# Glaciohound/Chimera-ST

Measured on AMD Instinct MI355X. Metric: train utterances/sec, MuST-C EN-DE s2t_transformer_m, 1/2/4/8 MI355X, higher is better.
Workload: dtype bf16

## Files before the change

chimera-st_amd/csrc/gemm.hip:

```cpp
#include "gemm_common.h"
#include <vector>
#include <stdlib.h>
#include <string>
#include <type_traits>

namespace {
using namespace cstg;

template <int BM_, int BN_, int WM_, int WN_, int KV_ = 8>
struct Cfg {
  static constexpr int BM = BM_, BN = BN_, WM = WM_, WN = WN_, NT = 64 * WM_ * WN_, TM = BM_ / WM_ / 32, TN = BN_ / WN_ / 32;
  static constexpr int KV = KV_;
  static_assert(BM_ <= GEMM_MAX_BM && GEMM_MAX_BM % BM_ == 0, "conv0.hip (cst_conv_row_limits) sizes live frames from GEMM_MAX_BM");
};
using CfgSmall = Cfg<128, 128, 2, 2>;
using CfgSkinny = Cfg<64, 64, 2, 2>;
using CfgNarrowN = Cfg<128, 64, 2, 2>;
using CfgNarrowM = Cfg<64, 128, 2, 2>;
using CfgLarge = Cfg<256, 256, 4, 4>;

template <typename T, bool A_KMAJOR, bool B_KMAJOR, bool SEG, typename C, bool CS = false>
__global__ __launch_bounds__(C::NT) void gemm_kernel(GemmParams p) {
  constexpr int BM = C::BM, BN = C::BN, NTHREADS = C::NT, TM = C::TM, TN = C::TN;
  constexpr int VEC = DT<T>::VEC;
// ... 698 lines not shown
      for (; sp < p.splits; ++sp) {
        const f32x4 a0 = *reinterpret_cast<const f32x4*>(src + (int64_t)sp * total), a1 = *reinterpret_cast<const f32x4*>(src + (int64_t)sp * total + 4);
#pragma unroll
        for (int e = 0; e < 4; ++e) { v[e] += a0[e]; v[4 + e] += a1[e]; }
      }
      const int64_t i = i8 * 8, row = i / p.N;
      epilogue_store8<T>(p, cofs, bofs, row, i - row * p.N, v);
    }
    return;
  }
  for (int64_t i = (int64_t)blockIdx.x * blockDim.x + threadIdx.x; i < total; i += (int64_t)gridDim.x * blockDim.x) {
    float v = 0.0f;
    for (int s = 0; s < p.splits; ++s) v += ws[s * total + i];
    epilogue_store<T>(p, cofs, bofs, i / p.N, i % p.N, v);
  }
}

template <typename T, bool AK, bool BK_, bool SEG, typename C>
int launch(GemmParams p, int64_t M, int64_t N, int64_t nbatch, hipStream_t s) {
  constexpr int VEC = DT<T>::VEC;
  constexpr int BKc = C::KV * VEC, LDK = BKc + VEC;
  constexpr int LDMA = sizeof(T) == 2 ? C::BM + 32 : C::BM + VEC, LDMB = sizeof(T) == 2 ? C::BN + 32 : C::BN + VEC;
  constexpr int A_ELEMS = AK ? C::BM * LDK : BKc * LDMA;
  constexpr int B_ELEMS = BK_ ? C::BN * LDK : BKc * LDMB;
  size_t lds = 2 * (size_t)(A_ELEMS + B_ELEMS) * sizeof(T);
  const size_t stage_bytes = (size_t)64 * (C::BN + 4) * sizeof(float);
  if (lds < stage_bytes) lds = stage_bytes;
  static bool attr_set = false;
  if (!attr_set) {
    (void)hipFuncSetAttribute(reinterpret_cast<const void*>(&gemm_kernel<T, AK, BK_, SEG, C>), hipFuncAttributeMaxDynamicSharedMemorySize, 160 * 1024 - 4096);
    attr_set = true;
  }
  p.tiles_m = (int)cst_ceil_div(M, C::BM);
  p.tiles_n = (int)cst_ceil_div(N, C::BN);
  static const bool no_split_order = getenv("CST_GEMM_NO_SPLIT_ORDER") != nullptr;
  p.split_order = (p.splits > 1 && nbatch == 1 && !no_split_order) ? 1 : 0;
  dim3 grid(p.tiles_m * p.tiles_n, 1, (unsigned)(nbatch * p.splits));
  if constexpr (!AK && !BK_ && !SEG && C::NT <= 256) {
    if (p.colsum) {
      static bool attr_cs = false;
      if (!attr_cs) {
        (void)hipFuncSetAttribute(reinterpret_cast<const void*>(&gemm_kernel<T, AK, BK_, SEG, C, true>), hipFuncAttributeMaxDynamicSharedMemorySize, 160 * 1024 - 4096);
        attr_cs = true;
      }
      hipLaunchKernelGGL((gemm_kernel<T, AK, BK_, SEG, C, true>), grid, dim3(C::NT), lds, s, p);
      return cst_check_launch("cst_gemm");
    }
  }
  if (p.colsum) { cst_set_error("cst_gemm: internal: column sums requested from a configuration that does not build them"); return CST_ERR_UNSUPPORTED; }
  hipLaunchKernelGGL((gemm_kernel<T, AK, BK_, SEG, C>), grid, dim3(C::NT), lds, s, p);
  return cst_check_launch("cst_gemm");
}

template <typename T, bool AK, bool BK_, typename C, int NS>
int launch_glds(GemmParams p, int64_t M, int64_t N, int64_t nbatch, hipStream_t s) {
  constexpr int ES = sizeof(T), BKc = 128 / ES;
  constexpr int A_BYTES = AK ? C::BM * 128 : BKc * C::BM * ES, B_BYTES = BK_ ? C::BN * 128 : BKc * C::BN * ES;
  size_t lds = (size_t)NS * (A_BYTES + B_BYTES);
  const size_t stage_bytes = (size_t)64 * (C::BN + 4) * sizeof(float);
  if (lds < stage_bytes) lds = stage_bytes;
  static bool attr_set = false;
  if (!attr_set) {
    (void)hipFuncSetAttribute(reinterpret_cast<const void*>(&gemm_glds_kernel<T, AK, BK_, C, NS>), hipFuncAttributeMaxDynamicSharedMemorySize, 160 * 1024);
    attr_set = true;
  }
  p.tiles_m = (int)cst_ceil_div(M, C::BM);
  p.tiles_n = (int)cst_ceil_div(N, C::BN);
  dim3 grid(p.tiles_m * p.tiles_n, 1, (unsigned)(nbatch * p.splits));
  hipLaunchKernelGGL((gemm_glds_kernel<T, AK, BK_, C, NS>), grid, dim3(C::NT), lds, s, p);
  return cst_check_launch("cst_gemm");
}

bool use_large(const cst_gemm_desc* d, int splits) {
  if ((d->a_kmajor && d->a_seg) || (d->b_kmajor && d->b_seg)) return false;
  const int64_t tiles = cst_ceil_div(d->M, 256) * cst_ceil_div(d->N, 256) * d->batch0 * d->batch1 * splits;
  return d->M >= 256 && d->N >= 256 && tiles >= 200;
}

bool getenv_no_glds() {
  static const bool v = getenv("CST_GEMM_NO_GLDS") != nullptr;
  return v;
}

int choose_splits(const cst_gemm_desc* d) {
  if (d->split_k > 1) return d->split_k;
  if (d->split_k == 0 || d->split_k == 1) return 1;
  const int bk = d->dtype == CST_BF16 ? 64 : 32;
  const int64_t ktiles = cst_ceil_div(d->K, bk);
  const int64_t nb = d->batch0 * d->batch1;
  if (d->M >= 256 && d->N >= 256) {
    const int64_t tl = cst_ceil_div(d->M, 256) * cst_ceil_div(d->N, 256) * nb;
    if (tl >= 200) return 1;
    int64_t s = 256 / tl;
    if (s > ktiles / 16) s = ktiles / 16;
    if (s > 32) s = 32;
    if (s >= 1 && tl * s >= 200) return (int)s;
  }
  const int64_t tiles = cst_ceil_div(d->M, 128) * cst_ceil_div(d->N, 128) * nb;
  if (tiles >= 256 || ktiles < 16) return 1;
  const int64_t cap = ktiles / 8 < 32 ? ktiles / 8 : 32;
  int64_t s1 = 256 / tiles, s2 = 512 / tiles;
  if (s1 > cap) s1 = cap;
  if (s2 > cap) s2 = cap;
  if (s1 < 1) s1 = 1;
  if (s2 < 1) s2 = 1;
  const int64_t s = (2.0 / (double)s2 < 0.9 / (double)s1) ? s2 : s1;
  return (int)s;
}

}

static bool colsum_fused(const cst_gemm_desc* d, int splits) {
  return d->colsum && !d->a_kmajor && !d->b_kmajor && !d->a_seg && !d->b_seg && !use_large(d, splits);
}

extern "C" int64_t cst_colsum_workspace(int64_t rows, int64_t cols);
extern "C" int cst_colsum_typed(const void* x, int64_t ldx, void* out, void* workspace, int64_t rows, int64_t cols, int dtype, int out_dtype, cst_stream stream);
extern "C" int cst_colsum_typed_live(const void* x, int64_t ldx, void* out, void* workspace, int64_t rows, int64_t cols, int dtype, int out_dtype,
                                     const uint32_t* row_live, uint32_t epoch, cst_stream stream);

extern "C" int cst_gemm_splits(const cst_gemm_desc* d) { return d ? choose_splits(d) : 0; }

extern "C" int cst_gemm_colsum_is_fused(const cst_gemm_desc* d) { return d && colsum_fused(d, choose_splits(d)) ? 1 : 0; }

extern "C" int64_t cst_gemm_workspace(const cst_gemm_desc* d) {
  const int s = choose_splits(d);
  const int64_t nb = d->batch0 * d->batch1;
  int64_t bytes = s > 1 ? (int64_t)s * d->M * d->N * nb * (int64_t)sizeof(float) : 0;
  if (d->colsum) bytes += colsum_fused(d, s) ? (s > 1 ? (int64_t)s * d->M * nb * (int64_t)sizeof(float) : 0) : cst_colsum_workspace(d->K, d->M);
  return bytes;
}

static int gemm_one(const cst_gemm_desc* d, cst_stream stream, int64_t drop_row0) {
  CST_REQUIRE(d && d->A && d->B && d->C, "cst_gemm: null operand");
  CST_REQUIRE(d->dtype == CST_F32 || d->dtype == CST_BF16, "cst_gemm: bad dtype %d", d->dtype);
  CST_REQUIRE(d->c_dtype == d->dtype || d->c_dtype == CST_F32, "cst_gemm: c_dtype must be dtype or f32");
  CST_REQUIRE(d->M > 0 && d->N > 0 && d->K > 0, "cst_gemm: empty problem M=%lld N=%lld K=%lld", (long long)d->M,
              (long long)d->N, (long long)d->K);
  const int vec = d->dtype == CST_BF16 ? 8 : 4;
  if (d->a_kmajor) CST_REQUIRE(d->K % vec == 0 && d->lda % vec == 0, "cst_gemm: k-major A needs K,lda %% %d == 0 (K=%lld lda=%lld)", vec, (long long)d->K, (long long)d->lda);
  else CST_REQUIRE(d->M % vec == 0 && d->lda % vec == 0, "cst_gemm: mn-major A needs M,lda %% %d == 0 (M=%lld lda=%lld)", vec, (long long)d->M, (long long)d->lda);
  if (d->b_kmajor) CST_REQUIRE(d->K % vec == 0 && d->ldb % vec == 0, "cst_gemm: k-major B needs K,ldb %% %d == 0 (K=%lld ldb=%lld)", vec, (long long)d->K, (long long)d->ldb);
  else CST_REQUIRE(d->N % vec == 0 && d->ldb % vec == 0, "cst_gemm: mn-major B needs N,ldb %% %d == 0 (N=%lld ldb=%lld)", vec, (long long)d->N, (long long)d->ldb);
  CST_REQUIRE(d->a_seg % vec == 0 && d->b_seg % vec == 0 && d->a_seg_stride % vec == 0 && d->b_seg_stride % vec == 0,
              "cst_gemm: segment sizes must be multiples of %d", vec);
  CST_REQUIRE(((uintptr_t)d->A % 16 == 0) && ((uintptr_t)d->B % 16 == 0), "cst_gemm: A/B must be 16-byte aligned");
  CST_REQUIRE(d->sa0 % vec == 0 && d->sa1 % vec == 0 && d->sb0 % vec == 0 && d->sb1 % vec == 0, "cst_gemm: batch strides of A/B must be multiples of %d", vec);
  CST_REQUIRE(d->batch0 >= 1 && d->batch1 >= 1, "cst_gemm: batch counts must be >= 1");
  CST_REQUIRE(!d->dact || d->aux_in, "cst_gemm: dact needs aux_in");

  GemmParams p;
  p.M = d->M; p.N = d->N; p.K = d->K;
  p.A = d->A; p.lda = d->lda; p.a_seg = d->a_seg; p.a_seg_stride = d->a_seg_stride;
  p.B = d->B; p.ldb = d->ldb; p.b_seg = d->b_seg; p.b_seg_stride = d->b_seg_stride;
  p.C = d->C; p.ldc = d->ldc;
  p.bias = d->bias; p.bias_mode = d->bias ? d->bias_mode : CST_BIAS_NONE; p.sbias0 = d->sbias0; p.sbias1 = d->sbias1;
  p.act = d->act;
  p.aux_out = d->aux_out; p.ld_aux_out = d->ld_aux_out;
  p.dact = d->dact; p.aux_in = d->aux_in; p.ld_aux_in = d->ld_aux_in;
  p.resid = d->resid; p.ld_resid = d->ld_resid;
  p.alpha = d->alpha;
  CST_REQUIRE(d->drop_p >= 0.0f && d->drop_p < 1.0f, "cst_gemm: drop_p must be in [0, 1)");
  CST_REQUIRE(d->drop_p == 0.0f || d->batch0 * d->batch1 == 1, "cst_gemm: fused dropout needs an unbatched problem");
  p.drop_thr = d->drop_p > 0.0f ? cst_drop_thr16(d->drop_p) : 0u;
  p.drop_key = d->drop_key;
  p.drop_scale = d->drop_p > 0.0f ? 1.0f / (1.0f - d->drop_p) : 1.0f;
  p.drop_row0 = drop_row0;
  p.batch1 = d->batch1;
  p.sa0 = d->sa0; p.sa1 = d->sa1; p.sb0 = d->sb0; p.sb1 = d->sb1; p.sc0 = d->sc0; p.sc1 = d->sc1;
  p.c_f32 = (d->c_dtype == CST_F32 && d->dtype != CST_F32) ? 1 : 0;
  if (d->dtype == CST_F32) p.c_f32 = 0;
  {
    auto al16 = [](const void* q) { return q == nullptr || ((uintptr_t)q % 16) == 0; };
    bool ok = d->ldc % 8 == 0 && d->sc0 % 8 == 0 && d->sc1 % 8 == 0 && al16(d->C) && al16(d->bias) && al16(d->aux_out) && al16(d->aux_in) && al16(d->resid);
    if (d->bias && d->bias_mode == CST_BIAS_COL) ok = ok && d->sbias0 % 8 == 0 && d->sbias1 % 8 == 0;
    if (d->aux_out) ok = ok && d->ld_aux_out % 8 == 0;
    if (d->aux_in) ok = ok && d->ld_aux_in % 8 == 0;
    if (d->resid) ok = ok && d->ld_resid % 8 == 0;
    if (d->drop_p > 0.0f) ok = ok && (d->N % 2 == 0);
    p.vec_epi = ok ? 1 : 0;
  }
  p.tiles_m = p.tiles_n = 0;
  p.split_order = 0;
  p.sched = nullptr;
  p.gperm_full = 0;
  p.mrot = 0;
  {
    static const bool no_klive = getenv("CST_GEMM_NO_KLIVE") != nullptr;
    p.k_live = no_klive ? nullptr : d->k_live;
    p.k_epoch = d->k_epoch;
    p.m_live = no_klive ? nullptr : d->m_live;
    p.m_epoch = d->m_epoch;
    p.k_len = no_klive ? nullptr : d->k_len;
    p.m_len = no_klive ? nullptr : d->m_len;
  }
  {
    static const int gm = getenv("CST_GEMM8P_GROUP_M") ? atoi(getenv("CST_GEMM8P_GROUP_M")) : 4;
    p.group_m = gm > 0 ? gm : 4;
  }
  p.splits = choose_splits(d);
  p.ws = nullptr;
  CST_REQUIRE(!d->colsum || (!d->a_kmajor && !d->a_seg), "cst_gemm: colsum needs an mn-major, unsegmented A");
  const bool cs_fused = colsum_fused(d, p.splits);
  CST_REQUIRE(!d->colsum || cs_fused || (d->batch0 * d->batch1 == 1 && d->M % 8 == 0 && d->lda % 8 == 0),
              "cst_gemm: colsum of this configuration runs as a separate column sum: unbatched, M and lda multiples of 8");
  p.colsum = cs_fused ? d->colsum : nullptr;
  p.colsum_ws = nullptr;
#ifdef CST_TRACE
  if (p.splits == 1 && d->workspace) p.ws = (float*)d->workspace;
#endif
  const int64_t nbatch = d->batch0 * d->batch1;
  CST_REQUIRE(cst_ceil_div(d->M, 128) * cst_ceil_div(d->N, 128) < (1ll << 31) && nbatch * p.splits < 65536, "cst_gemm: grid too large");
  if (p.splits > 1) {
    const int64_t need = cst_gemm_workspace(d);
    if (!d->workspace || d->workspace_bytes < need) {
      cst_set_error("cst_gemm: split_k=%d needs %lld workspace bytes, got %lld", p.splits, (long long)need,
                    (long long)d->workspace_bytes);
      return CST_ERR_WORKSPACE;
    }
    p.ws = (float*)d->workspace;
    p.colsum_ws = p.ws + (int64_t)p.splits * d->M * d->N * nbatch;
  } else if (d->colsum && !cs_fused && (!d->workspace || d->workspace_bytes < cst_gemm_workspace(d))) {
    cst_set_error("cst_gemm: colsum needs %lld workspace bytes, got %lld", (long long)cst_gemm_workspace(d), (long long)d->workspace_bytes);
    return CST_ERR_WORKSPACE;
  }
  hipStream_t s = (hipStream_t)stream;
  double kfrac = 1.0;
  if (p.k_live && cst_prof_is_on()) {
    const int64_t nt = cst_ceil_div(d->K, 64);
    std::vector<uint32_t> st((size_t)nt);
    if (hipStreamSynchronize(s) == hipSuccess && hipMemcpy(st.data(), p.k_live, sizeof(uint32_t) * nt, hipMemcpyDeviceToHost) == hipSuccess) {
      int64_t live = 0;
      for (int64_t i = 0; i < nt; ++i) live += st[i] == p.k_epoch;
      kfrac = (double)live / (double)nt;
    }
  }
  if (p.k_len && cst_prof_is_on()) {
    std::vector<int32_t> kl((size_t)d->batch0);
    if (hipStreamSynchronize(s) == hipSuccess && hipMemcpy(kl.data(), p.k_len, sizeof(int32_t) * d->batch0, hipMemcpyDeviceToHost) == hipSuccess) {
      double sum = 0.0;
      for (int64_t b = 0; b < d->batch0; ++b) sum += (double)(kl[b] < 0 ? 0 : (kl[b] < d->K ? kl[b] : d->K));
      kfrac *= sum / ((double)d->batch0 * (double)d->K);
    }
  }
  if (p.m_len && cst_prof_is_on()) {
    std::vector<int32_t> ml((size_t)d->batch0);
    if (hipStreamSynchronize(s) == hipSuccess && hipMemcpy(ml.data(), p.m_len, sizeof(int32_t) * d->batch0, hipMemcpyDeviceToHost) == hipSuccess) {
      const int64_t tiles = cst_ceil_div(d->M, 256);
      double live = 0.0;
      for (int64_t b = 0; b < d->batch0; ++b) {
        const int64_t t = ml[b] <= 0 ? 0 : cst_ceil_div((int64_t)ml[b], 256);
        live += (double)(t < tiles ? t : tiles);
      }
      kfrac *= live / ((double)d->batch0 * (double)tiles);
    }
  }
  if (p.m_live && cst_prof_is_on()) {
    const int64_t nt = cst_ceil_div(d->M, 64);
    std::vector<uint32_t> st((size_t)nt);
    if (hipStreamSynchronize(s) == hipSuccess && hipMemcpy(st.data(), p.m_live, sizeof(uint32_t) * nt, hipMemcpyDeviceToHost) == hipSuccess) {
      int64_t live = 0, tiles = cst_ceil_div(d->M, 256);
      for (int64_t t = 0; t < tiles; ++t) {
        bool l = false;
        for (int64_t i = 4 * t; i < 4 * t + 4 && i < nt; ++i) l |= st[i] == p.m_epoch;
        live += l;
      }
      kfrac *= (double)live / (double)tiles;
    }
  }
  const double flops = 2.0 * (double)d->M * (double)d->N * (double)d->K * (double)nbatch * kfrac;
  const double esz = (double)cst_dtype_size(d->dtype);
  const double bytes = ((double)d->M * d->K + (double)d->N * d->K) * esz * nbatch * kfrac + (double)d->M * d->N * cst_dtype_size(d->c_dtype) * nbatch;
  CstProfScope prof(CST_K_GEMM, s, flops, bytes);
  int rc;
  const bool ak = d->a_kmajor != 0, bk = d->b_kmajor != 0;
  const bool seg = (ak && d->a_seg) || (bk && d->b_seg);
  const bool large = use_large(d, p.splits);
#define CST_GEMM_LAYOUT(T, SEGV, CFG)                                                                                   \
  (ak ? (bk ? launch<T, true, true, SEGV, CFG>(p, d->M, d->N, nbatch, s) : launch<T, true, false, SEGV, CFG>(p, d->M, d->N, nbatch, s)) \
      : (bk ? launch<T, false, true, SEGV, CFG>(p, d->M, d->N, nbatch, s) : launch<T, false, false, SEGV, CFG>(p, d->M, d->N, nbatch, s)))
#define CST_GLDS_LAYOUT(T, CFG, NS)                                                                                     \
  (ak ? (bk ? launch_glds<T, true, true, CFG, NS>(p, d->M, d->N, nbatch, s) : launch_glds<T, true, false, CFG, NS>(p, d->M, d->N, nbatch, s)) \
      : (bk ? launch_glds<T, false, true, CFG, NS>(p, d->M, d->N, nbatch, s) : launch_glds<T, false, false, CFG, NS>(p, d->M, d->N, nbatch, s)))
  static const bool glds_all = getenv("CST_GEMM_GLDS_ALL") != nullptr;
  const bool no_glds = getenv_no_glds() || (!(ak && bk) && !glds_all) || d->colsum != nullptr;
#define CST_GEMM_DISPATCH(T)                                                                         \
  (seg ? CST_GEMM_LAYOUT(T, true, CfgSmall)                                                           \
       : (no_glds ? (large ? CST_GEMM_LAYOUT(T, false, CfgLarge) : CST_GEMM_LAYOUT(T, false, CfgSmall)) \
                  : (large ? CST_GLDS_LAYOUT(T, CfgLarge, 2) : CST_GLDS_LAYOUT(T, CfgSmall, 2))))
  static const bool no_8p = getenv("CST_GEMM_NO_8P") != nullptr, force_8p = getenv("CST_GEMM_FORCE_8P") != nullptr;
  static const bool all_8p = getenv("CST_GEMM_8P_ALL") != nullptr;
  static const bool dact_8p = getenv("CST_GEMM_8P_NO_DACT") == nullptr;
  static const bool no_skinny = getenv("CST_GEMM_NO_SKINNY") != nullptr;
  static const int64_t skinny_tiles = getenv("CST_GEMM_SKINNY_TILES") ? atoll(getenv("CST_GEMM_SKINNY_TILES")) : 256;
  static const bool skinny_ns4 = getenv("CST_GEMM_SKINNY_NS4") != nullptr;
  static const bool no_mid8p = getenv("CST_GEMM_NO_MID8P") != nullptr;
  const bool mid8p = !no_mid8p && ak && bk && !seg && nbatch == 1 && p.splits == 1 && d->M >= 256 && d->N >= 256 &&
                     cst_ceil_div(d->M, 256) * cst_ceil_div(d->N, 256) >= 150;
  static const bool no_narrow = getenv("CST_GEMM_NO_NARROW") != nullptr;
  static const bool no_4w = getenv("CST_GEMM_NO_4W") != nullptr;
  static const bool experiment = getenv("CST_GEMM_EXPERIMENT") != nullptr;
  const char* force_cfg = experiment ? getenv("CST_GEMM_FORCE_CFG") : nullptr;
  if (force_cfg && !*force_cfg) force_cfg = nullptr;
  if (!no_narrow && !seg && !large && ak && bk && d->N <= 64 && d->M > 256) {
    rc = d->dtype == CST_BF16 ? launch_glds<bf16_t, true, true, CfgNarrowN, 2>(p, d->M, d->N, nbatch, s)
                              : launch_glds<float, true, true, CfgNarrowN, 2>(p, d->M, d->N, nbatch, s);
  } else if (!no_narrow && !seg && !large && !ak && !bk && d->M <= 64 && d->N > 256) {
    rc = d->dtype == CST_BF16 ? launch<bf16_t, false, false, false, CfgNarrowM>(p, d->M, d->N, nbatch, s)
                              : launch<float, false, false, false, CfgNarrowM>(p, d->M, d->N, nbatch, s);
  } else if (force_cfg && !ak && !bk && !seg && nbatch == 1 && d->dtype == CST_BF16) {
    const std::string f(force_cfg);
    if (f == "small") rc = launch<bf16_t, false, false, false, CfgSmall>(p, d->M, d->N, nbatch, s);
    else if (f == "narrowm") rc = launch<bf16_t, false, false, false, CfgNarrowM>(p, d->M, d->N, nbatch, s);
    else if (f == "narrown") rc = launch<bf16_t, false, false, false, CfgNarrowN>(p, d->M, d->N, nbatch, s);
    else if (f == "skinny") rc = launch<bf16_t, false, false, false, CfgSkinny>(p, d->M, d->N, nbatch, s);
    else if (f == "large") rc = launch<bf16_t, false, false, false, CfgLarge>(p, d->M, d->N, nbatch, s);
    else if (f == "big4r") rc = launch<bf16_t, false, false, false, Cfg<256, 256, 2, 2>>(p, d->M, d->N, nbatch, s);
    else { cst_set_error("cst_gemm: unknown CST_GEMM_FORCE_CFG %s", force_cfg); return CST_ERR_BAD_ARG; }
  } else if (force_cfg && ak && bk && !seg && nbatch == 1 && p.splits == 1 && d->dtype == CST_BF16) {
    const std::string f(force_cfg);
    if (f == "skinny4") rc = launch_glds<bf16_t, true, true, CfgSkinny, 4>(p, d->M, d->N, nbatch, s);
    else if (f == "skinny2") rc = launch_glds<bf16_t, true, true, CfgSkinny, 2>(p, d->M, d->N, nbatch, s);
    else if (f == "small2") rc = launch_glds<bf16_t, true, true, CfgSmall, 2>(p, d->M, d->N, nbatch, s);
    else if (f == "small3") rc = launch_glds<bf16_t, true, true, CfgSmall, 3>(p, d->M, d->N, nbatch, s);
    else if (f == "big4") rc = launch_glds<bf16_t, true, true, Cfg<256, 256, 2, 2>, 2>(p, d->M, d->N, nbatch, s);
    else if (f == "big4n") rc = launch_glds<bf16_t, true, true, Cfg<256, 192, 2, 2>, 2>(p, d->M, d->N, nbatch, s);
    else if (f == "big4r") rc = launch<bf16_t, true, true, false, Cfg<256, 256, 2, 2>>(p, d->M, d->N, nbatch, s);
    else if (f == "large") rc = launch<bf16_t, true, true, false, CfgLarge>(p, d->M, d->N, nbatch, s);
    else if (f == "8p" && cst_gemm8p_supported(p, ak, bk, nbatch)) rc = cst_gemm8p_launch(p, ak, bk, nbatch, s);
    else if (f == "4w" && cst_gemm4w_supported(p, ak, bk, nbatch)) rc = cst_gemm4w_launch(p, s);
    else { cst_set_error("cst_gemm: unknown CST_GEMM_FORCE_CFG %s", force_cfg); return CST_ERR_BAD_ARG; }
  } else if (!no_skinny && ak && bk && !seg && nbatch == 1 && p.splits == 1 &&
             (d->M <= 256 || (!large && !mid8p && cst_ceil_div(d->M, 128) * cst_ceil_div(d->N, 128) < skinny_tiles))) {
    const bool two_stage = d->M > 256 && cst_ceil_div(d->M, 64) * cst_ceil_div(d->N, 64) > 512 && !skinny_ns4;
    if (two_stage) rc = d->dtype == CST_BF16 ? launch_glds<bf16_t, true, true, CfgSkinny, 2>(p, d->M, d->N, nbatch, s)
                                             : launch_glds<float, true, true, CfgSkinny, 2>(p, d->M, d->N, nbatch, s);
    else rc = d->dtype == CST_BF16 ? launch_glds<bf16_t, true, true, CfgSkinny, 4>(p, d->M, d->N, nbatch, s)
                                   : launch_glds<float, true, true, CfgSkinny, 4>(p, d->M, d->N, nbatch, s);
  } else if (d->dtype == CST_BF16 && !seg && !no_4w && !d->colsum && cst_gemm4w_supported(p, ak, bk, nbatch)) {
    rc = cst_gemm4w_launch(p, s);
  } else if (d->dtype == CST_BF16 && !seg && !no_8p && !d->colsum && (ak || all_8p || force_8p) && (!d->dact || (dact_8p && !d->resid && !d->aux_out) || all_8p || force_8p) && (large || mid8p || force_8p) && cst_gemm8p_supported(p, ak, bk, nbatch))
    rc = cst_gemm8p_launch(p, ak, bk, nbatch, s);
  else if (d->dtype == CST_BF16) rc = CST_GEMM_DISPATCH(bf16_t);
  else rc = CST_GEMM_DISPATCH(float);
#undef CST_GEMM_DISPATCH
#undef CST_GEMM_LAYOUT
#undef CST_GLDS_LAYOUT
  if (cst_prof_is_on())
    prof.tag("M=%lld N=%lld K=%lld b=%lld a%c b%c split=%d%s%s%s%s%s%s%s", (long long)d->M, (long long)d->N, (long long)d->K, (long long)nbatch, ak ? 'k' : 'm',
             bk ? 'k' : 'm', p.splits, d->bias ? " bias" : "", d->act ? " act" : "", d->aux_out ? " aux_out" : "", d->dact ? " dact" : "",
             d->resid ? " resid" : "", d->drop_p > 0 ? " drop" : "", (d->k_live || d->m_live || d->k_len || d->m_len) ? " live" : "");
  if (rc != CST_OK) return rc;
  if (p.splits > 1 && d->defer_reduce) {
    CST_REQUIRE((nbatch == 1 || !d->colsum) && d->alpha == 1.0f && !d->bias && !d->act && !d->dact && !d->aux_out && !d->resid && d->drop_p == 0.0f && d->ldc == d->N &&
                    d->N % 8 == 0 && (!d->colsum || cs_fused),
                "cst_gemm: defer_reduce needs a plain epilogue and a dense C (batched: no colsum; the slabs are [batch][split][M][N])");
    return rc;
  }
  if (p.splits > 1) {
    const int64_t total = d->M * d->N;
    const int64_t work = (p.vec_epi && d->N % 8 == 0) ? total / 8 : total;
    int blocks = (int)(cst_ceil_div(work, 256) < 2048 ? cst_ceil_div(work, 256) : 2048);
    dim3 grid(blocks, (unsigned)nbatch);
    if (d->dtype == CST_BF16) hipLaunchKernelGGL(splitk_reduce_kernel<bf16_t>, grid, dim3(256), 0, s, p);
    else hipLaunchKernelGGL(splitk_reduce_kernel<float>, grid, dim3(256), 0, s, p);
    rc = cst_check_launch("cst_gemm split-k reduce");
  }
  if (rc == CST_OK && d->colsum && !cs_fused) {
    void* cws = (char*)d->workspace + (p.splits > 1 ? (int64_t)p.splits * d->M * d->N * (int64_t)sizeof(float) : 0);
    rc = p.k_live ? cst_colsum_typed_live(d->A, d->lda, d->colsum, cws, d->K, d->M, d->dtype, d->dtype, p.k_live, p.k_epoch, stream)
                  : cst_colsum_typed(d->A, d->lda, d->colsum, cws, d->K, d->M, d->dtype, d->dtype, stream);
  }
  return rc;
}

extern "C" int cst_gemm(const cst_gemm_desc* d, cst_stream stream) { return gemm_one(d, stream, 0); }
```

chimera-st_amd/csrc/gemm4w.hip:

```cpp
#include "gemm_common.h"
#include <cstdlib>

namespace {
using namespace cstg;
using T = bf16_t;
using u32x2 = __attribute__((ext_vector_type(2))) unsigned int;

constexpr int BM = 256, TN = 3, BN = 64 * TN, BK = 64, NT = 256;
static_assert(BM <= cstg::GEMM_MAX_BM && cstg::GEMM_MAX_BM % BM == 0, "conv0.hip (cst_conv_row_limits) sizes live frames from GEMM_MAX_BM");
constexpr int IMGA = BM * 128, IMGB = BN * 128;
constexpr int NSA = 3, NSB = 2;
constexpr int BOFF = NSA * IMGA;
constexpr int GA = BM / 32, GB = BN / 32, G = GA + GB;
constexpr int NSLOT = 2 * TN, NFR = 4 + TN;
constexpr int ERS = 2 * (BN / 2) + 16;
constexpr int LDS_BYTES = NSA * IMGA + NSB * IMGB > 4 * 128 * ERS ? NSA * IMGA + NSB * IMGB : 4 * 128 * ERS;

__global__ __launch_bounds__(NT) void gemm4w_kernel(GemmParams p) {
  extern __shared__ __attribute__((aligned(16))) char smem[];
  const int tid = threadIdx.x, lane = tid & 63, wave = tid >> 6;
  const int wm = wave >> 1, wn = wave & 1;
  const int lrow = lane & 31, hi = lane >> 5;
  const int ntiles = p.tiles_m * p.tiles_n;
  int id = blockIdx.x;
  {
    const int q = ntiles / 8, r = ntiles % 8, xcd = id % 8, loc = id / 8;
    id = (xcd < r ? xcd * (q + 1) : r * (q + 1) + (xcd - r) * q) + loc;
  }
  const int GROUP_M = p.group_m;
  const int per_group = GROUP_M * p.tiles_n;
  const int grp = id / per_group, rem = id % per_group;
  const int gm0 = grp * GROUP_M;
  const int gsz = (p.tiles_m - gm0 < GROUP_M) ? (p.tiles_m - gm0) : GROUP_M;
  const int tm = gm0 + rem % gsz, tn = rem / gsz;
  const int64_t m0 = (int64_t)tm * BM, n0 = (int64_t)tn * BN;
  const int mrem = (int)(p.M - m0 < BM ? p.M - m0 : BM);

  int nkt = (int)(p.K / BK);
  if (p.m_live) {
    typedef const __attribute__((address_space(4))) uint32_t* cptr_t;
    cptr_t ml = (cptr_t)p.m_live;
    const int t0 = (int)(m0 >> 6), tnn = (int)((p.M + 63) >> 6);
    bool live = false;
#pragma unroll
    for (int i = 0; i < 4; ++i) live |= (t0 + i < tnn) && ml[t0 + i < tnn ? t0 + i : t0] == p.m_epoch;
    if (!live) nkt = 0;
  }

  const int row0 = 8 * wave + (lane >> 3);
  const unsigned lda2 = (unsigned)(p.lda * 2), ldb2 = (unsigned)(p.ldb * 2);
  const unsigned chs = (unsigned)(((lane & 7) ^ ((row0 >> 1) & 7)) << 4);
  const unsigned voffa = (unsigned)row0 * lda2 + chs, voffb = (unsigned)row0 * ldb2 + chs;
  const __amdgpu_buffer_rsrc_t rsA = __builtin_amdgcn_make_buffer_rsrc((void*)((const T*)p.A + m0 * p.lda), (short)0,
                                                                         (int)((unsigned)(mrem - 1) * lda2 + (unsigned)(p.K * 2)), 0x00020000);
  const __amdgpu_buffer_rsrc_t rsB = __builtin_amdgcn_make_buffer_rsrc((void*)((const T*)p.B + n0 * p.ldb), (short)0,
                                                                         (int)((unsigned)(BN - 1) * ldb2 + (unsigned)(p.K * 2)), 0x00020000);
  auto dma_a = [&](int i, int kt, int stg) {
    char* dst = smem + stg * IMGA + (wave + 4 * i) * 1024;
    __builtin_amdgcn_raw_ptr_buffer_load_lds(rsA, (__attribute__((address_space(3))) void*)dst, 16, (int)voffa,
                                             (int)((unsigned)(32 * i) * lda2 + (unsigned)kt * 128u), 0, 0);
  };
  auto dma_b = [&](int i, int kt, int stg) {
    char* dst = smem + BOFF + stg * IMGB + (wave + 4 * i) * 1024;
    __builtin_amdgcn_raw_ptr_buffer_load_lds(rsB, (__attribute__((address_space(3))) void*)dst, 16, (int)voffb,
                                             (int)((unsigned)(32 * i) * ldb2 + (unsigned)kt * 128u), 0, 0);
  };
  const int swr = (lrow >> 1) & 7;
  const unsigned fa0 = (unsigned)((wm * 128 + lrow) * 128), fb0 = (unsigned)(BOFF + (wn * 32 * TN + lrow) * 128);
  unsigned fch[4];
#pragma unroll
  for (int kk = 0; kk < 4; ++kk) fch[kk] = (unsigned)(((2 * kk + hi) ^ swr) << 4);

  f32x16 acc[4][TN];
  if (p.bias_mode == CST_BIAS_COL) {
#pragma unroll
    for (int j = 0; j < TN; ++j)
#pragma unroll
      for (int q = 0; q < 4; ++q) {
        const u32x2 raw = *reinterpret_cast<const u32x2*>((const T*)p.bias + n0 + wn * 32 * TN + j * 32 + 8 * q + 4 * hi);
        const float b0 = __uint_as_float(raw[0] << 16), b1 = __uint_as_float(raw[0] & 0xffff0000u);
        const float b2 = __uint_as_float(raw[1] << 16), b3 = __uint_as_float(raw[1] & 0xffff0000u);
#pragma unroll
        for (int i = 0; i < 4; ++i) { acc[i][j][4 * q] = b0; acc[i][j][4 * q + 1] = b1; acc[i][j][4 * q + 2] = b2; acc[i][j][4 * q + 3] = b3; }
      }
  } else {
#pragma unroll
    for (int i = 0; i < 4; ++i)
#pragma unroll
      for (int j = 0; j < TN; ++j)
#pragma unroll
        for (int r = 0; r < 16; ++r) acc[i][j][r] = 0.0f;
  }

  if (nkt > 0) {
#pragma unroll
    for (int i = 0; i < GA; ++i) dma_a(i, 0, 0);
#pragma unroll
    for (int i = 0; i < GB; ++i) dma_b(i, 0, 0);
    if (nkt > 1) {
#pragma unroll
      for (int i = 0; i < GA; ++i) dma_a(i, 1, 1);
    }
  }
  bf16x8 fa[2][4], fb[2][TN];
  int sa = 0;
  for (int kt = 0; kt < nkt; ++kt) {
    const int sb = kt & 1;
    if (kt + 1 < nkt) asm volatile("s_waitcnt vmcnt(8) lgkmcnt(0)" ::: "memory");
    else asm volatile("s_waitcnt vmcnt(0) lgkmcnt(0)" ::: "memory");
    __builtin_amdgcn_s_barrier();
    const char* abase = smem + sa * IMGA;
    const char* bbase = smem + sb * IMGB;
    auto read_one = [&](int f, int kk, int nb) {
      if (f < 4) fa[nb][f] = *reinterpret_cast<const bf16x8*>(abase + fa0 + f * 4096 + fch[kk]);
      else fb[nb][f - 4] = *reinterpret_cast<const bf16x8*>(bbase + fb0 + (f - 4) * 4096 + fch[kk]);
    };
#pragma unroll
    for (int f = 0; f < NFR; ++f) read_one(f, 0, 0);
    __builtin_amdgcn_sched_barrier(0);
    const bool more_b = kt + 1 < nkt, more_a = kt + 2 < nkt;
    const int sa2 = sa == 0 ? 2 : sa - 1;
#pragma unroll
    for (int kk = 0; kk < 4; ++kk) {
#pragma unroll
      for (int sl = 0; sl < NSLOT; ++sl) {
#pragma unroll
        for (int u = 0; u < 2; ++u) {
          const int m = 2 * sl + u, i = m / TN, j = m % TN;
          acc[i][j] = __builtin_amdgcn_mfma_f32_32x32x16_bf16(fb[kk & 1][j], fa[kk & 1][i], acc[i][j], 0, 0, 0);
        }
        if (kk < 3) {
          if (sl < NFR) read_one(sl, kk + 1, (kk + 1) & 1);
          if (sl == 0) read_one(NSLOT, kk + 1, (kk + 1) & 1);
        }
        {
          const int d = kk * NSLOT + sl;
          if (d < GB) { if (more_b) dma_b(d, kt + 1, sb ^ 1); }
          else if (d < G) { if (more_a) dma_a(d - GB, kt + 2, sa2); }
        }
        __builtin_amdgcn_sched_barrier(0);
      }
    }
    sa = sa == 2 ? 0 : sa + 1;
  }
  static_assert(NFR == NSLOT + 1, "the slot plan above places exactly one extra fragment read");

  constexpr int CPR = BN / 2 / 8;
  constexpr int NPC = 128 * CPR / 64;
  const int64_t rbase_m = m0 + wm * 128, cbase_n = n0 + wn * (BN / 2);
  const T* resid = (const T*)p.resid;
  u32x4 exq[NPC];
  if (resid) {
#pragma unroll
    for (int t = 0; t < NPC; ++t) {
      const int v = t * 64 + lane, rl = v / CPR, cl = (v % CPR) * 8;
      int64_t row = rbase_m + rl;
      row = row < p.M ? row : p.M - 1;
      exq[t] = __builtin_nontemporal_load(reinterpret_cast<const u32x4*>(resid + row * p.ld_resid + cbase_n + cl));
    }
  }
  __syncthreads();
  {
    char* img = smem + wave * (128 * ERS);
#pragma unroll
    for (int i = 0; i < 4; ++i)
#pragma unroll
      for (int j = 0; j < TN; ++j)
#pragma unroll
        for (int q = 0; q < 4; ++q) {
          typedef __bf16 bf16x4_t __attribute__((ext_vector_type(4)));
          bf16x4_t pk;
#pragma unroll
          for (int e = 0; e < 4; ++e) pk[e] = static_cast<__bf16>(acc[i][j][4 * q + e] * p.alpha);
          *reinterpret_cast<u32x2*>(img + (i * 32 + lrow) * ERS + (j * 32 + 8 * q + 4 * hi) * 2) = __builtin_bit_cast(u32x2, pk);
        }
    asm volatile("s_waitcnt lgkmcnt(0)" ::: "memory");
    if (p.drop_thr || resid) {
#pragma unroll
      for (int t = 0; t < NPC; ++t) {
        const int v = t * 64 + lane, rl = v / CPR, cl = (v % CPR) * 8;
        const int64_t row = rbase_m + rl, col = cbase_n + cl;
        const u32x4 zraw = *reinterpret_cast<const u32x4*>(img + rl * ERS + cl * 2);
        float x[8];
#pragma unroll
        for (int e = 0; e < 4; ++e) {
          x[2 * e] = __uint_as_float(zraw[e] << 16);
          x[2 * e + 1] = __uint_as_float(zraw[e] & 0xffff0000u);
        }
        if (p.drop_thr) cst_drop8(x, p.drop_key, (uint64_t)((row + p.drop_row0) * p.N + col), p.drop_thr, p.drop_scale);
        if (resid) {
#pragma unroll
          for (int e = 0; e < 4; ++e) {
            x[2 * e] += __uint_as_float(exq[t][e] << 16);
            x[2 * e + 1] += __uint_as_float(exq[t][e] & 0xffff0000u);
          }
        }
        bf16x8 ob;
#pragma unroll
        for (int e = 0; e < 8; ++e) ob[e] = static_cast<__bf16>(x[e]);
        *reinterpret_cast<u32x4*>(img + rl * ERS + cl * 2) = __builtin_bit_cast(u32x4, ob);
      }
    }
#pragma unroll 8
    for (int t = 0; t < NPC; ++t) {
      const int v = t * 64 + lane, rl = v / CPR, cl = (v % CPR) * 8;
      const int64_t row = rbase_m + rl;
      if (row >= p.M) continue;
      const u32x4 o = *reinterpret_cast<const u32x4*>(img + rl * ERS + cl * 2);
      __builtin_nontemporal_store(o, reinterpret_cast<u32x4*>((T*)p.C + row * p.ldc + cbase_n + cl));
    }
  }
}
}

bool cst_gemm4w_supported(const cstg::GemmParams& p, bool ak, bool bk, int64_t nbatch) {
  if (!ak || !bk || nbatch != 1 || p.splits != 1 || p.c_f32 || !p.vec_epi) return false;
  if (p.N % BN || p.K % BK || p.K < 1536 || p.M < 256) return false;
  if (p.a_seg || p.b_seg || p.act || p.aux_out || p.dact || p.m_len) return false;
  if (p.bias_mode != CST_BIAS_NONE && (p.bias_mode != CST_BIAS_COL || p.alpha != 1.0f)) return false;
  if (p.lda * 2 * 256 + p.K * 2 >= (1ll << 31) || p.ldb * 2 * 256 >= (1ll << 31)) return false;
  const int64_t tiles = cst_ceil_div(p.M, BM) * (p.N / BN);
  const int64_t r = tiles % 256;
  static const int64_t max_tiles = [] { const char* e = getenv("CST_GEMM_4W_MAXTILES"); return e ? (int64_t)atoll(e) : (int64_t)768; }();
  return tiles >= 256 && tiles <= max_tiles && (r == 0 || r >= (tiles > 512 ? 170 : 115));
}

int cst_gemm4w_launch(cstg::GemmParams p, hipStream_t s) {
  static bool attr_set = false;
  if (!attr_set) {
    (void)hipFuncSetAttribute(reinterpret_cast<const void*>(&gemm4w_kernel), hipFuncAttributeMaxDynamicSharedMemorySize, LDS_BYTES);
    attr_set = true;
  }
  p.tiles_m = (int)cst_ceil_div(p.M, BM);
  p.tiles_n = (int)(p.N / BN);
  static const int group_m = [] { const char* e = getenv("CST_GEMM_4W_GROUP_M"); const int g = e ? atoi(e) : 8; return g > 0 ? g : 8; }();
  p.group_m = group_m;
  hipLaunchKernelGGL(gemm4w_kernel, dim3((unsigned)(p.tiles_m * p.tiles_n)), dim3(NT), LDS_BYTES, s, p);
  return cst_check_launch("cst_gemm (4-wave)");
}
```

chimera-st_amd/csrc/gemm_common.h:

```cpp
#pragma once
#include "cst_common.h"

namespace cstg {

constexpr int GEMM_MAX_BM = 256;

struct GemmParams {
  int64_t M, N, K;
  const void* A; int64_t lda, a_seg, a_seg_stride;
  const void* B; int64_t ldb, b_seg, b_seg_stride;
  void* C; int64_t ldc;
  const void* bias; int bias_mode; int64_t sbias0, sbias1;
  int act;
  void* aux_out; int64_t ld_aux_out;
  int dact;
  const void* aux_in; int64_t ld_aux_in;
  const void* resid; int64_t ld_resid;
  float alpha;
  uint32_t drop_thr, drop_key; float drop_scale;
  int64_t drop_row0;
  int64_t batch1;
  int64_t sa0, sa1, sb0, sb1, sc0, sc1;
  int splits;
  float* ws;
  int c_f32;
  int vec_epi;
  int tiles_m, tiles_n;
  int nz;
  int half_from, nitems;
  int group_m;
  unsigned long long magic_ntiles, magic_per_group;
  int per_group, group_shift;
  int gperm_full, gperm_q, gperm_r;
  int mrot;
  unsigned long long magic_gq, magic_gq1;
  int split_order;
  int* sched;
  const uint32_t* m_live; uint32_t m_epoch;
  const int32_t* k_len;
  const int32_t* m_len;
  const uint32_t* k_live; uint32_t k_epoch;
  void* colsum;
  float* colsum_ws;
};

__device__ __forceinline__ int64_t segaddr(int64_t c, int64_t seg, int64_t seg_stride) {
  return seg ? (c / seg) * seg_stride + (c % seg) : c;
}

template <typename T>
__device__ __forceinline__ void epilogue_store(const GemmParams& p, int64_t cofs, int64_t bofs, int64_t row, int64_t col, float v) {
  v *= p.alpha;
  if (p.bias_mode == CST_BIAS_COL) v += DT<T>::ld((const T*)p.bias + bofs + col);
  else if (p.bias_mode == CST_BIAS_ROW) v += DT<T>::ld((const T*)p.bias + bofs + row);
  if (p.aux_out) DT<T>::st((T*)p.aux_out + cofs + row * p.ld_aux_out + col, v);
  v = act_t<T>(v, p.act);
  if (p.drop_thr) v *= cst_drop1(p.drop_key, (uint64_t)((row + p.drop_row0) * p.N + col), p.drop_thr, p.drop_scale);
  if (p.dact) v *= dact_t<T>(DT<T>::ld((const T*)p.aux_in + cofs + row * p.ld_aux_in + col), p.dact);
  if (p.resid) v += DT<T>::ld((const T*)p.resid + cofs + row * p.ld_resid + col);
  if (p.c_f32) ((float*)p.C)[cofs + row * p.ldc + col] = v;
  else DT<T>::st((T*)p.C + cofs + row * p.ldc + col, v);
}

template <typename T>
__device__ __forceinline__ void epilogue_store8(const GemmParams& p, int64_t cofs, int64_t bofs, int64_t row, int64_t col, float (&v)[8]) {
#pragma unroll
  for (int e = 0; e < 8; ++e) v[e] *= p.alpha;
  if (p.bias_mode == CST_BIAS_COL) {
    float b[8];
    load8((const T*)p.bias + bofs + col, b);
#pragma unroll
    for (int e = 0; e < 8; ++e) v[e] += b[e];
  } else if (p.bias_mode == CST_BIAS_ROW) {
    const float b = DT<T>::ld((const T*)p.bias + bofs + row);
#pragma unroll
    for (int e = 0; e < 8; ++e) v[e] += b;
  }
  if (p.aux_out) store8((T*)p.aux_out + cofs + row * p.ld_aux_out + col, v);
  if (p.act == CST_ACT_RELU) {
#pragma unroll
    for (int e = 0; e < 8; ++e) v[e] = fmaxf(v[e], 0.0f);
  } else if (p.act == CST_ACT_GELU) {
#pragma unroll
    for (int e = 0; e < 8; ++e) v[e] = gelu_t<T>(v[e]);
  }
  if (p.drop_thr) cst_drop8(v, p.drop_key, (uint64_t)((row + p.drop_row0) * p.N + col), p.drop_thr, p.drop_scale);
  if (p.dact) {
    float z[8];
    load8((const T*)p.aux_in + cofs + row * p.ld_aux_in + col, z);
#pragma unroll
    for (int e = 0; e < 8; ++e) v[e] *= dact_t<T>(z[e], p.dact);
  }
  if (p.resid) {
    float r[8];
    load8((const T*)p.resid + cofs + row * p.ld_resid + col, r);
#pragma unroll
    for (int e = 0; e < 8; ++e) v[e] += r[e];
  }
  if (p.c_f32) store8((float*)p.C + cofs + row * p.ldc + col, v);
  else store8((T*)p.C + cofs + row * p.ldc + col, v);
}

}

int cst_gemm8p_launch(cstg::GemmParams p, bool a_kmajor, bool b_kmajor, int64_t nbatch, hipStream_t s);
bool cst_gemm8p_supported(const cstg::GemmParams& p, bool a_kmajor, bool b_kmajor, int64_t nbatch);
int cst_gemm4w_launch(cstg::GemmParams p, hipStream_t s);
bool cst_gemm4w_supported(const cstg::GemmParams& p, bool a_kmajor, bool b_kmajor, int64_t nbatch);
```

Before: 507.0.

## Extend 4-wave GEMM to K>=768, act/aux_out and dact epilogues with prefetch

The 4-wave GEMM kernel is templated on an epilogue mode (residual, activation/aux_out, dact) and gains an option that prefetches the residual or aux_in tile during the last two K iterations. Support widens to K>=768 and to fused activation and dact epilogues. Default dispatch now also goes through a new preferred check, which still excludes act/aux_out/dact cases but allows K in [768,1536) for plain or residual GEMMs. The aim is to use the faster kernel on more mid-size GEMMs and to hide epilogue load latency, at the cost of more template instances and code complexity.

```diff
diff --git a/chimera-st_amd/csrc/gemm.hip b/chimera-st_amd/csrc/gemm.hip
--- a/chimera-st_amd/csrc/gemm.hip
+++ b/chimera-st_amd/csrc/gemm.hip
@@ -1024,6 +1024,7 @@
   static const bool experiment = getenv("CST_GEMM_EXPERIMENT") != nullptr;
   const char* force_cfg = experiment ? getenv("CST_GEMM_FORCE_CFG") : nullptr;
   if (force_cfg && !*force_cfg) force_cfg = nullptr;
+  if (force_cfg && std::string(force_cfg) == "4w" && !(d->dtype == CST_BF16 && cst_gemm4w_supported(p, ak, bk, nbatch))) force_cfg = nullptr;
   if (!no_narrow && !seg && !large && ak && bk && d->N <= 64 && d->M > 256) {
     rc = d->dtype == CST_BF16 ? launch_glds<bf16_t, true, true, CfgNarrowN, 2>(p, d->M, d->N, nbatch, s)
                               : launch_glds<float, true, true, CfgNarrowN, 2>(p, d->M, d->N, nbatch, s);
@@ -1059,7 +1060,7 @@
                                              : launch_glds<float, true, true, CfgSkinny, 2>(p, d->M, d->N, nbatch, s);
     else rc = d->dtype == CST_BF16 ? launch_glds<bf16_t, true, true, CfgSkinny, 4>(p, d->M, d->N, nbatch, s)
                                    : launch_glds<float, true, true, CfgSkinny, 4>(p, d->M, d->N, nbatch, s);
-  } else if (d->dtype == CST_BF16 && !seg && !no_4w && !d->colsum && cst_gemm4w_supported(p, ak, bk, nbatch)) {
+  } else if (d->dtype == CST_BF16 && !seg && !no_4w && !d->colsum && cst_gemm4w_supported(p, ak, bk, nbatch) && cst_gemm4w_preferred(p)) {
     rc = cst_gemm4w_launch(p, s);
   } else if (d->dtype == CST_BF16 && !seg && !no_8p && !d->colsum && (ak || all_8p || force_8p) && (!d->dact || (dact_8p && !d->resid && !d->aux_out) || all_8p || force_8p) && (large || mid8p || force_8p) && cst_gemm8p_supported(p, ak, bk, nbatch))
     rc = cst_gemm8p_launch(p, ak, bk, nbatch, s);
diff --git a/chimera-st_amd/csrc/gemm4w.hip b/chimera-st_amd/csrc/gemm4w.hip
--- a/chimera-st_amd/csrc/gemm4w.hip
+++ b/chimera-st_amd/csrc/gemm4w.hip
@@ -1,5 +1,6 @@
 #include "gemm_common.h"
 #include <cstdlib>
+#include <type_traits>
 
 namespace {
 using namespace cstg;
@@ -16,6 +17,7 @@
 constexpr int ERS = 2 * (BN / 2) + 16;
 constexpr int LDS_BYTES = NSA * IMGA + NSB * IMGB > 4 * 128 * ERS ? NSA * IMGA + NSB * IMGB : 4 * 128 * ERS;
 
+template <int EPI, bool PRE>
 __global__ __launch_bounds__(NT) void gemm4w_kernel(GemmParams p) {
   extern __shared__ __attribute__((aligned(16))) char smem[];
   const int tid = threadIdx.x, lane = tid & 63, wave = tid >> 6;
@@ -71,6 +73,27 @@
 #pragma unroll
   for (int kk = 0; kk < 4; ++kk) fch[kk] = (unsigned)(((2 * kk + hi) ^ swr) << 4);
 
+  constexpr int CPR = BN / 2 / 8;
+  constexpr int NPC = 128 * CPR / 64;
+  const int64_t rbase_m = m0 + wm * 128, cbase_n = n0 + wn * (BN / 2);
+  const T* exsrc = EPI == 2 ? (const T*)p.aux_in : (EPI == 0 ? (const T*)p.resid : nullptr);
+  const int64_t exld = EPI == 2 ? p.ld_aux_in : p.ld_resid;
+  const bool zero_tile = EPI != 0 && nkt == 0 && p.bias_mode == CST_BIAS_NONE && !p.resid;
+  u32x4 exq[NPC];
+  using I0 = std::integral_constant<int, 0>;
+  using I1 = std::integral_constant<int, 1>;
+  using I2 = std::integral_constant<int, 2>;
+  auto ex_req = [&](auto hc) {
+    constexpr int H = decltype(hc)::value;
+#pragma unroll
+    for (int t = H * (NPC / 2); t < (H + 1) * (NPC / 2); ++t) {
+      const int v = t * 64 + lane, rl = v / CPR, cl = (v % CPR) * 8;
+      int64_t row = rbase_m + rl;
+      row = row < p.M ? row : p.M - 1;
+      exq[t] = __builtin_nontemporal_load(reinterpret_cast<const u32x4*>(exsrc + row * exld + cbase_n + cl));
+    }
+  };
+
   f32x16 acc[4][TN];
   if (p.bias_mode == CST_BIAS_COL) {
 #pragma unroll
@@ -104,7 +127,8 @@
   }
   bf16x8 fa[2][4], fb[2][TN];
   int sa = 0;
-  for (int kt = 0; kt < nkt; ++kt) {
+  auto ktile = [&](const int kt, auto phc) {
+    constexpr int PH = decltype(phc)::value;
     const int sb = kt & 1;
     if (kt + 1 < nkt) asm volatile("s_waitcnt vmcnt(8) lgkmcnt(0)" ::: "memory");
     else asm volatile("s_waitcnt vmcnt(0) lgkmcnt(0)" ::: "memory");
@@ -118,6 +142,10 @@
 #pragma unroll
     for (int f = 0; f < NFR; ++f) read_one(f, 0, 0);
     __builtin_amdgcn_sched_barrier(0);
+    if constexpr (PH != 0) {
+      if (exsrc) ex_req(std::integral_constant<int, PH - 1>{});
+      __builtin_amdgcn_sched_barrier(0);
+    }
     const bool more_b = kt + 1 < nkt, more_a = kt + 2 < nkt;
     const int sa2 = sa == 0 ? 2 : sa - 1;
 #pragma unroll
@@ -142,40 +170,89 @@
       }
     }
     sa = sa == 2 ? 0 : sa + 1;
+  };
+  if constexpr (PRE) {
+    for (int kt = 0; kt < nkt - 2; ++kt) ktile(kt, I0{});
+    if (nkt >= 2) ktile(nkt - 2, I1{});
+    if (nkt >= 1) ktile(nkt - 1, I2{});
+  } else {
+    for (int kt = 0; kt < nkt; ++kt) ktile(kt, I0{});
   }
   static_assert(NFR == NSLOT + 1, "the slot plan above places exactly one extra fragment read");
 
-  constexpr int CPR = BN / 2 / 8;
-  constexpr int NPC = 128 * CPR / 64;
-  const int64_t rbase_m = m0 + wm * 128, cbase_n = n0 + wn * (BN / 2);
-  const T* resid = (const T*)p.resid;
-  u32x4 exq[NPC];
-  if (resid) {
-#pragma unroll
+  if constexpr (EPI != 0) {
+    if (zero_tile) {
+      const u32x4 z4 = {0u, 0u, 0u, 0u};
+#pragma unroll 8
+      for (int t = 0; t < NPC; ++t) {
+        const int v = t * 64 + lane, rl = v / CPR, cl = (v % CPR) * 8;
+        const int64_t row = rbase_m + rl;
+        if (row >= p.M) continue;
+        __builtin_nontemporal_store(z4, reinterpret_cast<u32x4*>((T*)p.C + row * p.ldc + cbase_n + cl));
+        if (EPI == 1 && p.aux_out) __builtin_nontemporal_store(z4, reinterpret_cast<u32x4*>((T*)p.aux_out + row * p.ld_aux_out + cbase_n + cl));
+      }
+      return;
+    }
+  }
+
+  if (exsrc) {
+    if constexpr (PRE) {
+      if (nkt < 2) ex_req(I0{});
+      if (nkt < 1) ex_req(I1{});
+    } else {
+      ex_req(I0{});
+      ex_req(I1{});
+    }
+  }
+  __syncthreads();
+  char* img = smem + wave * (128 * ERS);
+#pragma unroll
+  for (int i = 0; i < 4; ++i)
+#pragma unroll
+    for (int j = 0; j < TN; ++j)
+#pragma unroll
+      for (int q = 0; q < 4; ++q) {
+        typedef __bf16 bf16x4_t __attribute__((ext_vector_type(4)));
+        bf16x4_t pk;
+#pragma unroll
+        for (int e = 0; e < 4; ++e) pk[e] = static_cast<__bf16>(acc[i][j][4 * q + e] * p.alpha);
+        *reinterpret_cast<u32x2*>(img + (i * 32 + lrow) * ERS + (j * 32 + 8 * q + 4 * hi) * 2) = __builtin_bit_cast(u32x2, pk);
+      }
+  asm volatile("s_waitcnt lgkmcnt(0)" ::: "memory");
+  if constexpr (EPI == 1) {
+    const bool post = p.act != CST_ACT_NONE || p.drop_thr;
+#pragma unroll 4
     for (int t = 0; t < NPC; ++t) {
       const int v = t * 64 + lane, rl = v / CPR, cl = (v % CPR) * 8;
-      int64_t row = rbase_m + rl;
-      row = row < p.M ? row : p.M - 1;
-      exq[t] = __builtin_nontemporal_load(reinterpret_cast<const u32x4*>(resid + row * p.ld_resid + cbase_n + cl));
-    }
-  }
-  __syncthreads();
-  {
-    char* img = smem + wave * (128 * ERS);
-#pragma unroll
-    for (int i = 0; i < 4; ++i)
-#pragma unroll
-      for (int j = 0; j < TN; ++j)
-#pragma unroll
-        for (int q = 0; q < 4; ++q) {
-          typedef __bf16 bf16x4_t __attribute__((ext_vector_type(4)));
-          bf16x4_t pk;
-#pragma unroll
-          for (int e = 0; e < 4; ++e) pk[e] = static_cast<__bf16>(acc[i][j][4 * q + e] * p.alpha);
-          *reinterpret_cast<u32x2*>(img + (i * 32 + lrow) * ERS + (j * 32 + 8 * q + 4 * hi) * 2) = __builtin_bit_cast(u32x2, pk);
-        }
-    asm volatile("s_waitcnt lgkmcnt(0)" ::: "memory");
-    if (p.drop_thr || resid) {
+      const int64_t row = rbase_m + rl, col = cbase_n + cl;
+      if (row >= p.M) continue;
+      const u32x4 zraw = *reinterpret_cast<const u32x4*>(img + rl * ERS + cl * 2);
+      if (p.aux_out) __builtin_nontemporal_store(zraw, reinterpret_cast<u32x4*>((T*)p.aux_out + row * p.ld_aux_out + col));
+      u32x4 o = zraw;
+      if (post) {
+        float x[8];
+#pragma unroll
+        for (int e = 0; e < 4; ++e) {
+          x[2 * e] = __uint_as_float(zraw[e] << 16);
+          x[2 * e + 1] = __uint_as_float(zraw[e] & 0xffff0000u);
+        }
+        if (p.act == CST_ACT_RELU) {
+#pragma unroll
+          for (int e = 0; e < 8; ++e) x[e] = fmaxf(x[e], 0.0f);
+        } else if (p.act == CST_ACT_GELU) {
+#pragma unroll
+          for (int e = 0; e < 8; ++e) x[e] = gelu_t<T>(x[e]);
+        }
+        if (p.drop_thr) cst_drop8(x, p.drop_key, (uint64_t)((row + p.drop_row0) * p.N + col), p.drop_thr, p.drop_scale);
+        bf16x8 ob;
+#pragma unroll
+        for (int e = 0; e < 8; ++e) ob[e] = static_cast<__bf16>(x[e]);
+        o = __builtin_bit_cast(u32x4, ob);
+      }
+      __builtin_nontemporal_store(o, reinterpret_cast<u32x4*>((T*)p.C + row * p.ldc + col));
+    }
+  } else {
+    if (p.drop_thr || exsrc) {
 #pragma unroll
       for (int t = 0; t < NPC; ++t) {
         const int v = t * 64 + lane, rl = v / CPR, cl = (v % CPR) * 8;
@@ -188,11 +265,16 @@
           x[2 * e + 1] = __uint_as_float(zraw[e] & 0xffff0000u);
         }
         if (p.drop_thr) cst_drop8(x, p.drop_key, (uint64_t)((row + p.drop_row0) * p.N + col), p.drop_thr, p.drop_scale);
-        if (resid) {
+        if (exsrc) {
 #pragma unroll
           for (int e = 0; e < 4; ++e) {
-            x[2 * e] += __uint_as_float(exq[t][e] << 16);
-            x[2 * e + 1] += __uint_as_float(exq[t][e] & 0xffff0000u);
+            if constexpr (EPI == 2) {
+              x[2 * e] *= dact_t<T>(__uint_as_float(exq[t][e] << 16), p.dact);
+              x[2 * e + 1] *= dact_t<T>(__uint_as_float(exq[t][e] & 0xffff0000u), p.dact);
+            } else {
+              x[2 * e] += __uint_as_float(exq[t][e] << 16);
+              x[2 * e + 1] += __uint_as_float(exq[t][e] & 0xffff0000u);
+            }
           }
         }
         bf16x8 ob;
@@ -211,30 +293,49 @@
     }
   }
 }
+
+template <int EPI, bool PRE>
+int launch4w(const GemmParams& p, hipStream_t s) {
+  static bool attr_set = false;
+  if (!attr_set) {
+    (void)hipFuncSetAttribute(reinterpret_cast<const void*>(&gemm4w_kernel<EPI, PRE>), hipFuncAttributeMaxDynamicSharedMemorySize, LDS_BYTES);
+    attr_set = true;
+  }
+  hipLaunchKernelGGL((gemm4w_kernel<EPI, PRE>), dim3((unsigned)(p.tiles_m * p.tiles_n)), dim3(NT), LDS_BYTES, s, p);
+  return cst_check_launch("cst_gemm (4-wave)");
+}
 }
 
 bool cst_gemm4w_supported(const cstg::GemmParams& p, bool ak, bool bk, int64_t nbatch) {
   if (!ak || !bk || nbatch != 1 || p.splits != 1 || p.c_f32 || !p.vec_epi) return false;
-  if (p.N % BN || p.K % BK || p.K < 1536 || p.M < 256) return false;
-  if (p.a_seg || p.b_seg || p.act || p.aux_out || p.dact || p.m_len) return false;
+  if (p.N % BN || p.K % BK || p.K < 768 || p.M < 256) return false;
+  if (p.a_seg || p.b_seg || p.m_len) return false;
+  if (p.dact && (!p.aux_in || p.act || p.aux_out || p.resid)) return false;
+  if ((p.act || p.aux_out) && p.resid) return false;
   if (p.bias_mode != CST_BIAS_NONE && (p.bias_mode != CST_BIAS_COL || p.alpha != 1.0f)) return false;
   if (p.lda * 2 * 256 + p.K * 2 >= (1ll << 31) || p.ldb * 2 * 256 >= (1ll << 31)) return false;
+  return true;
+}
+
+bool cst_gemm4w_preferred(const cstg::GemmParams& p) {
   const int64_t tiles = cst_ceil_div(p.M, BM) * (p.N / BN);
   const int64_t r = tiles % 256;
+  if (p.act || p.aux_out || p.dact) return false;
+  if (p.K < 1536) {
+    static const bool no_k768 = getenv("CST_GEMM_4W_NO_K768") != nullptr;
+    if (no_k768) return false;
+  }
   static const int64_t max_tiles = [] { const char* e = getenv("CST_GEMM_4W_MAXTILES"); return e ? (int64_t)atoll(e) : (int64_t)768; }();
   return tiles >= 256 && tiles <= max_tiles && (r == 0 || r >= (tiles > 512 ? 170 : 115));
 }
 
 int cst_gemm4w_launch(cstg::GemmParams p, hipStream_t s) {
-  static bool attr_set = false;
-  if (!attr_set) {
-    (void)hipFuncSetAttribute(reinterpret_cast<const void*>(&gemm4w_kernel), hipFuncAttributeMaxDynamicSharedMemorySize, LDS_BYTES);
-    attr_set = true;
-  }
   p.tiles_m = (int)cst_ceil_div(p.M, BM);
   p.tiles_n = (int)(p.N / BN);
   static const int group_m = [] { const char* e = getenv("CST_GEMM_4W_GROUP_M"); const int g = e ? atoi(e) : 8; return g > 0 ? g : 8; }();
   p.group_m = group_m;
-  hipLaunchKernelGGL(gemm4w_kernel, dim3((unsigned)(p.tiles_m * p.tiles_n)), dim3(NT), LDS_BYTES, s, p);
-  return cst_check_launch("cst_gemm (4-wave)");
-}
+  if (p.dact) return launch4w<2, true>(p, s);
+  if (p.act || p.aux_out) return launch4w<1, false>(p, s);
+  if (p.resid && p.K < 1536) return launch4w<0, true>(p, s);
+  return launch4w<0, false>(p, s);
+}
diff --git a/chimera-st_amd/csrc/gemm_common.h b/chimera-st_amd/csrc/gemm_common.h
--- a/chimera-st_amd/csrc/gemm_common.h
+++ b/chimera-st_amd/csrc/gemm_common.h
@@ -107,3 +107,4 @@
 bool cst_gemm8p_supported(const cstg::GemmParams& p, bool a_kmajor, bool b_kmajor, int64_t nbatch);
 int cst_gemm4w_launch(cstg::GemmParams p, hipStream_t s);
 bool cst_gemm4w_supported(const cstg::GemmParams& p, bool a_kmajor, bool b_kmajor, int64_t nbatch);
+bool cst_gemm4w_preferred(const cstg::GemmParams& p);
```

Measured after the change: 504.0, median of 4. No clear change (-0.6%).
